# Iamdarika/Spotify_recommender

Measured on AMD Instinct MI355X. Metric: queries/sec, cosine top-100 over a 10M x 12 fp32 catalogue, higher is better.
Workload: dtype f32 (every score is the exact fp32 chain; a 12 B/row 8-bit replica only rules rows out); 1 GPU; 10000000 synthetic tracks x 12 fp32 features, top-100, 1 MI355X (BASELINE configs[2], HBM-roofline run); rows=10000000, topn=100, rows_per_gpu=10000000, lanes=2, seed=12345, generator=torch.rand(seed) uniform[0,1) on device

## Files before the change

spotify_recommender_amd/csrc/engine_single.hip.h:

```cpp
#pragma once

#include "engine_state.hip.h"

#include <type_traits>

namespace {

int flush_mstream(mi355rec* h, hipStream_t s);

bool use_half(const mi355rec* h, const uint64_t* upper_dev) {
    if (!h->d_half || upper_dev || h->replica_mode == MI355REC_REPLICA_OFF) return false;
    return h->replica_mode == MI355REC_REPLICA_ON || h->replica_mode == MI355REC_REPLICA_FP16 || h->n >= kHalfAutoMinRows;
}

bool use_q8(const mi355rec* h) { return h->d_q8 && h->replica_mode != MI355REC_REPLICA_FP16; }

int single_kind(const mi355rec* h, const uint64_t* upper_dev) {
    if (!use_half(h, upper_dev)) return kFp32;
    return use_q8(h) ? kQ8 : kFp16;
}

bool q8_exact_sample(const mi355rec* h) { return h->geom[kQ8].iters >= 3; }

constexpr int kBucketAutoMaxTopn = 128;
// ... 219 lines not shown
        L.epoch = next_epoch(h);
        if (enqueue_f32_seed(h, qptr, query12, exclude_global, topn, h->d_half_seed, h->d_lone_ctl, &h->lone_ctl_done, L.epoch, s))
            L.bound = &h->d_lone_ctl->cutoff;
        L.sample = h->d_half_seed;
    }
    const int rc = launch_scan(h, L, qptr, query12, exclude_global, topn, s);
    if (rc == MI355REC_OK && fused) *fused = L.tail.counters != nullptr;
    return rc;
}

int enqueue_merge(mi355rec* h, const uint64_t* lists, int n_lists, int list_len, int topn,
                  uint64_t* out_keys, int64_t* out_idx, float* out_score, hipStream_t s, uint32_t notify = 0) {
    const int slot = timing_begin(h, h->ev_merge, h->n_merge_pairs, h->merge_launches, s);
    hipLaunchKernelGGL(merge_kernel, dim3(1), dim3(kMergeBlock), 0, s, lists, n_lists, list_len,
                       static_cast<int64_t>(list_len), static_cast<int64_t>(0), topn, out_keys, out_idx, out_score,
                       static_cast<int64_t>(0), notify ? h->hd_done : static_cast<uint32_t*>(nullptr), notify);
    timing_end(h, h->ev_merge, h->n_merge_pairs, slot, s);
    HIP_TRY(h, hipGetLastError());
    return MI355REC_OK;
}

int check_topn(mi355rec* h, int topn, bool allow_rounds) {
    if (topn <= 0)
        return fail(h, MI355REC_ERR_INVALID_ARG, "topn must be positive, got %d", topn);
    if (!allow_rounds && topn > kMaxTopK)
        return fail(h, MI355REC_ERR_INVALID_ARG, "topn %d > %d is not supported by this call", topn, kMaxTopK);
    return MI355REC_OK;
}

bool pairs_open(const mi355rec* h);
int flush_streamed(mi355rec* h, hipStream_t s);
int enqueue_query(mi355rec* h, const float* qptr, const float* query12, int64_t exclude_global,
                  int topn_asked, uint64_t* out_keys, int64_t* out_idx, float* out_score, hipStream_t s, uint32_t notify = 0) {
    if (pairs_open(h)) {
        const int rc = flush_streamed(h, s);
        if (rc) return rc;
    }
    const int topn = static_cast<int64_t>(topn_asked) < h->n ? topn_asked : static_cast<int>(h->n);
    if (topn < topn_asked) {
        const size_t pad = static_cast<size_t>(topn_asked - topn);
        HIP_TRY(h, hipMemsetAsync(out_keys + topn, 0, pad * sizeof(uint64_t), s));
        if (out_idx) HIP_TRY(h, hipMemsetAsync(out_idx + topn, 0xff, pad * sizeof(int64_t), s));
        if (out_score) HIP_TRY(h, hipMemsetAsync(out_score + topn, 0, pad * sizeof(float), s));
    }
    for (int done = 0; done < topn; done += kMaxTopK) {
        const int k = topn - done < kMaxTopK ? topn - done : kMaxTopK;
        const uint64_t* upper = done ? out_keys + done - 1 : nullptr;
        int lists = 0;
        LoneTail lone{h->d_lone_ctr, out_keys, out_idx, out_score, h->hd_done, notify, {0u, 0u, 0u, 0u, 0u, 0u, 0u, 0u, 0u}};
        bool fused = false;
        int rc = enqueue_scan(h, qptr, query12, exclude_global, k, upper, s, &lists, (notify && h->d_lone_ctr) ? &lone : nullptr, &fused);
        if (rc) return rc;
        if (fused) {
            ++h->lone_fused;
            continue;
        }
        rc = enqueue_merge(h, h->d_block_lists, lists, k, k, out_keys + done,
                           out_idx ? out_idx + done : nullptr, out_score ? out_score + done : nullptr, s, notify);
        if (rc) return rc;
    }
    return MI355REC_OK;
}

int wait_done(mi355rec* h, uint32_t want) {
    for (uint64_t spins = 1;; ++spins) {
        if (__atomic_load_n(h->h_done, __ATOMIC_ACQUIRE) == want) return MI355REC_OK;
        __builtin_ia32_pause();
        if ((spins & 0x3ffff) == 0) {
            const hipError_t e = hipStreamQuery(h->stream);
            if (e == hipSuccess) {
                if (__atomic_load_n(h->h_done, __ATOMIC_ACQUIRE) == want) return MI355REC_OK;
                return fail(h, MI355REC_ERR_HIP, "the query's stream drained without its completion word");
            }
            if (e != hipErrorNotReady) return fail(h, MI355REC_ERR_HIP, "hipStreamQuery: %s", hipGetErrorString(e));
        }
    }
}

int ensure_streamed_alloc(mi355rec* h);
int ensure_streamed(mi355rec* h) {
    if (h->streamed_ready) return MI355REC_OK;
    const int rc = ensure_streamed_alloc(h);
    if (rc != MI355REC_OK) {
        for (int i = 0; i < 2; ++i) {
            if (h->d_stream_lists[i]) (void)hipFree(h->d_stream_lists[i]);
            h->d_stream_lists[i] = nullptr;
        }
        return rc;
    }
    h->streamed_ready = true;
    return MI355REC_OK;
}

int ensure_streamed_alloc(mi355rec* h) {
    const size_t words = static_cast<size_t>(most(h, &ScanGeom::sgrid)) * kMaxTopK;
    for (int i = 0; i < 2; ++i) HIP_TRY(h, hipMalloc(&h->d_stream_lists[i], sizeof(uint64_t) * words));
    return MI355REC_OK;
}

int merge_pending(mi355rec* h, hipStream_t s) {
    h->pending = false;
    return enqueue_merge(h, h->d_stream_lists[h->pending_buf], h->pending_lists, h->pending_topn, h->pending_topn,
                         h->pending_out, nullptr, nullptr, s);
}

int launch_stashed(mi355rec* h, hipStream_t s, bool with_next, const float* next_ptr, const float* next_q,
                   int64_t next_exclude, int next_topn, int next_buf, uint32_t next_epoch_tag);

int drain_pairs(mi355rec* h, hipStream_t s);

int flush_single_stream(mi355rec* h, hipStream_t s);
int flush_streamed(mi355rec* h, hipStream_t s) {
    const int rc = drain_pairs(h, s);
    return rc ? rc : flush_single_stream(h, s);
}

int flush_single_stream(mi355rec* h, hipStream_t s) {
    if (h->stashed.has) {
        const int rc = launch_stashed(h, s, false, nullptr, nullptr, -1, 0, 0, 0u);
        if (rc) return rc;
    }
    return h->pending ? merge_pending(h, s) : MI355REC_OK;
}

int launch_stashed(mi355rec* h, hipStream_t s, bool with_next, const float* next_ptr, const float* next_q,
                   int64_t next_exclude, int next_topn, int next_buf, uint32_t next_epoch_tag) {
    auto& st = h->stashed;
    const bool next_bucketed = with_next && use_bucket(h, st.kind, next_topn, h->geom_bucket.riders > 0);
    const ScanGeom& g = stream_geom(h, st.kind, next_bucketed);
    if (st.kind == kFp32 && h->pending && h->pending_topn > kRideTopnMax) {
        const int rc = merge_pending(h, s);
        if (rc) return rc;
    }
    ScanLaunch L;
    L.kind = st.kind;
    L.streamed = true;
    const int buf = h->pending ? 1 - h->pending_buf : 0;
    if (h->pending) L.prev = PrevMerge{h->d_stream_lists[h->pending_buf], h->pending_lists, h->pending_topn, h->pending_out};
    int scanners = g.sgrid;
    L.iters = g.siters;
    if (with_next && (g.riders > 0 || g.nbhd)) {
        scanners = g.r_scan;
        L.iters = g.r_iters;
        L.next = make_next_seed(h, st.kind, g.riders, g.nbhd, next_ptr, next_q, next_exclude, next_topn, next_epoch_tag,
                                h->d_stream_seed[next_buf], g.hoists ? h->d_stream_ctl + next_buf : nullptr, h->ctl_done[next_buf],
                                next_bucketed);
    }
    L.grid = scanners + 1 + L.next.n_wgs + L.next.nbhd;
    L.lists = h->d_stream_lists[buf];
    L.sample = h->d_stream_seed[st.seed_buf];
    L.bound = st.cutoff_ready ? &h->d_stream_ctl[st.seed_buf].cutoff : nullptr;
    L.epoch = st.epoch;
    L.bucketed = st.bucketed;
    const int rc = launch_scan(h, L, st.qptr, st.q, st.exclude, st.topn, s);
    if (rc) return rc;
    if (L.next.ctl) h->ctl_done[next_buf] += static_cast<unsigned>(L.next.n_wgs);
    h->pending = true;
    h->pending_buf = buf;
    h->pending_topn = st.topn;
    h->pending_out = st.out;
    h->pending_lists = scanners;
    st.has = false;
    return MI355REC_OK;
}

int enqueue_streamed_single(mi355rec* h, const float* qptr, const float* query12, int64_t exclude_global, int topn,
                            uint64_t* out_keys, hipStream_t s, int accepted_kind = -1) {
    int rc = MI355REC_OK;
    if (MI355REC_EXP_FLAG("MI355REC_EXP_RIDE_NOMERGE") && h->pending) {
        rc = flush_single_stream(h, s);
        if (rc) return rc;
    }
    const int kind = accepted_kind >= 0 ? accepted_kind : single_kind(h, nullptr);
    int seed_buf = 0;
    bool sampled = false, nbhd_taken = false;
    const uint32_t epoch = next_epoch(h);
    const bool bucketed = use_bucket(h, kind, topn, h->stashed.has && h->stashed.kind == kind && h->geom_bucket.riders > 0);
    const ScanGeom& ng = stream_geom(h, kind, bucketed);
    if (kind == kQ8) h->last_sample = bucketed ? MI355REC_SAMPLE_BUCKETED : MI355REC_SAMPLE_STRIDED;
    if (h->stashed.has) {
        seed_buf = 1 - h->stashed.seed_buf;
        const bool same = h->stashed.kind == kind;
        sampled = same && ng.riders > 0;
        nbhd_taken = same && ng.nbhd;
        rc = launch_stashed(h, s, same, qptr, query12, exclude_global, topn, seed_buf, epoch);
        if (rc) return rc;
    }
    bool bound_ready = sampled && ng.hoists;
    if (!sampled) {
        if (kind == kFp32) {
            if (h->n >= kF32LoneSeedMinRows)
                bound_ready = enqueue_f32_seed(h, qptr, query12, exclude_global, topn, h->d_stream_seed[seed_buf], h->d_stream_ctl + seed_buf,
                                               &h->ctl_done[seed_buf], epoch, s);
        } else if (!nbhd_taken) {
            enqueue_half_seed(h, kind, qptr, query12, exclude_global, topn, h->d_stream_seed[seed_buf], epoch, s, bucketed);
        }
        HIP_TRY(h, hipGetLastError());
    }
    auto& st = h->stashed;
    st.has = true;
    st.qptr = qptr;
    if (!qptr) std::memcpy(st.q, query12, sizeof st.q);
    st.exclude = exclude_global;
    st.topn = topn;
    st.out = out_keys;
    st.seed_buf = seed_buf;
    st.epoch = epoch;
    st.kind = kind;
    st.bucketed = bucketed;
    st.cutoff_ready = bound_ready;
    return MI355REC_OK;
}

bool pairing_on(const mi355rec* h) {
    if (h->pairing == MI355REC_PAIRING_ON || h->pairing == MI355REC_PAIRING_GROUPS) return true;
    if (h->pairing == MI355REC_PAIRING_OFF) return false;
    return h->n >= MI355REC_PAIRING_AUTO_MIN_ROWS;
}
bool groups_on(const mi355rec* h) {
    if (h->pairing == MI355REC_PAIRING_GROUPS) return true;
    return h->pairing == MI355REC_PAIRING_AUTO && h->n >= MI355REC_GROUPS_AUTO_MIN_ROWS;
}
bool pairs_open(const mi355rec* h) { return h->pairs.n_wait > 0 || h->pairs.n_form > 0 || h->pairs.n_pending > 0; }

void free_pairs(mi355rec* h) {
    auto& P = h->pairs;
    for (int i = 0; i < 8; ++i) {
        if (P.lists[i]) (void)hipFree(P.lists[i]);
        if (P.seed[i]) (void)hipFree(P.seed[i]);
        P.lists[i] = nullptr;
        P.seed[i] = nullptr;
    }
    if (P.ctl) (void)hipFree(P.ctl);
    P.ctl = nullptr;
    P.ready = false;
}

int ensure_pairs_alloc(mi355rec* h) {
    auto& P = h->pairs;
    const size_t words = static_cast<size_t>(h->geom[kQ8].grid > 0 ? h->geom[kQ8].grid : 1) * kPairMaxTopk;
    for (int i = 0; i < 8; ++i) {
        HIP_TRY(h, hipMalloc(&P.lists[i], sizeof(uint64_t) * words));
        HIP_TRY(h, hipMalloc(&P.seed[i], sizeof(unsigned long long) * kSampleSlots));
        HIP_TRY(h, hipMemset(P.seed[i], 0, sizeof(unsigned long long) * kSampleSlots));
    }
    HIP_TRY(h, hipMalloc(&P.ctl, sizeof(SeedCtl) * 8));
    HIP_TRY(h, hipMemset(P.ctl, 0, sizeof(SeedCtl) * 8));
    return MI355REC_OK;
}
int ensure_pairs(mi355rec* h) {
    if (h->pairs.ready) return MI355REC_OK;
    const int rc = ensure_pairs_alloc(h);
    if (rc != MI355REC_OK) {
        free_pairs(h);
        return rc;
    }
    for (unsigned& d : h->pairs.ctl_done) d = 0u;
    h->pairs.ready = true;
    return MI355REC_OK;
}

int merge_pair_pending(mi355rec* h, hipStream_t s) {
    auto& P = h->pairs;
    const int count = P.n_pending;
    P.n_pending = 0;
    for (int x = 0; x < count; ++x) {
        const int rc = enqueue_merge(h, P.lists[4 * P.pending_set + x], P.pending_lists, P.pending_topn, P.pending_topn, P.pending_out[x],
                                     nullptr, nullptr, s);
        if (rc) return rc;
    }
    return MI355REC_OK;
}

int launch_pairs(mi355rec* h, hipStream_t s, const mi355rec::Stashed* next, int n_next, bool next_bucketed) {
    auto& P = h->pairs;
    const int n_scan = P.n_wait;
    const int pairs = n_scan / 2;
    const int topn = P.wait[0].topn;
    if (P.n_pending) {
        bool shared = false;
        for (int x = 0; x < P.n_pending; ++x)
            for (int y = x + 1; y < P.n_pending; ++y) {
                const uint64_t* lo = P.pending_out[x] < P.pending_out[y] ? P.pending_out[x] : P.pending_out[y];
                const uint64_t* hi = P.pending_out[x] < P.pending_out[y] ? P.pending_out[y] : P.pending_out[x];
                shared = shared || hi < lo + P.pending_topn;
            }
        if (shared) {
            const int rc = merge_pair_pending(h, s);
            if (rc) return rc;
        }
    }
    const int side_queries = (pairs == 2 || P.n_pending == 4 || n_next == 4) ? 4 : 2;
    const ScanGeom& g = stream_geom(h, kQ8, n_next > 0 && next_bucketed);
    const bool riders = n_next > 0 && (g.riders > 0 || g.nbhd);
    const int extra = side_queries * (1 + (riders ? g.riders + (g.nbhd ? 1 : 0) : 0));
    const int64_t tiles = (h->n + Q8PairConfig::kTileRows - 1) / Q8PairConfig::kTileRows;
    int64_t slots = pairs == 2 ? (g.cap - extra) / 2 : g.grid - extra;
    if (slots > kRideMaxLists - 1) slots = kRideMaxLists - 1;
    if (slots > tiles) slots = tiles;
    if (pairs == 2 && slots >= 8) slots &= ~static_cast<int64_t>(7);
    if (slots < 1) slots = 1;
    const int64_t scanners = slots * pairs;
    const int iters = static_cast<int>((tiles + slots - 1) / slots);
    const int set = P.n_pending ? 1 - P.pending_set : 0;
    Q8PairSide side;
    std::memset(&side, 0, sizeof side);
    side.queries = side_queries;
    for (int x = 0; x < 4; ++x) side.prev[x] = no_prev_merge();
    for (int x = 0; x < P.n_pending; ++x)
        side.prev[x] = PrevMerge{P.lists[4 * P.pending_set + x], P.pending_lists, P.pending_topn, P.pending_out[x]};
    if (riders) {
        for (int x = 0; x < n_next; ++x)
            side.next[x] = make_next_seed(h, kQ8, g.riders, g.nbhd, next[x].qptr, next[x].q, next[x].exclude, next[x].topn, next[x].epoch,
                                          P.seed[next[x].seed_buf], g.hoists ? P.ctl + next[x].seed_buf : nullptr,
                                          P.ctl_done[next[x].seed_buf], next_bucketed);
        for (int x = n_next; x < side_queries; ++x) {
            side.next[x].n_wgs = side.next[0].n_wgs;
            side.next[x].nbhd = side.next[0].nbhd;
        }
    }
    Q8PairArgs args;
    std::memset(&args, 0, sizeof args);
    for (int x = 0; x < n_scan; ++x) {
        const mi355rec::Stashed& q = P.wait[x];
        Q8PairArg& a = args.q[x];
        a.qarg = make_query_arg(h, q.qptr, q.q);
        a.query_ptr = q.qptr;
        a.exclude_global = q.exclude;
        a.block_lists = P.lists[4 * set + x];
        a.seed_vals = P.seed[q.seed_buf];
        a.cutoff_ready = q.cutoff_ready ? &P.ctl[q.seed_buf].cutoff : nullptr;
        a.n_seed = q8_seed_count(h, q.bucketed);
        a.epoch = q.epoch;
    }
    const dim3 grid(static_cast<unsigned>(scanners + side_queries * (1 + side.next[0].n_wgs + side.next[0].nbhd)));
    LAUNCH_TIMED(h, h->ev_scan, h->n_scan_pairs, h->scan_launches, scan_q8_kernel_pair<Q8PairConfig>, grid, dim3(Q8PairConfig::kBlock), s,
                 h->d_feats, h->d_q8, h->n, iters, h->row_base, args, pairs, topn, h->d_half_rescored, side);
    HIP_TRY(h, hipGetLastError());
    h->half_scans += n_scan;
    h->q8_scans += n_scan;
    h->routes.q8 += n_scan;
    h->stream_pair_launches += pairs;
    if (pairs == 2) ++h->stream_group_launches;
    for (int x = 0; x < n_next; ++x)
        if (side.next[x].ctl) P.ctl_done[next[x].seed_buf] += static_cast<unsigned>(side.next[x].n_wgs);
    P.n_pending = n_scan;
    P.pending_set = set;
    P.pending_lists = static_cast<int>(slots);
    P.pending_topn = topn;
    for (int x = 0; x < n_scan; ++x) P.pending_out[x] = P.wait[x].out;
    P.n_wait = 0;
    return MI355REC_OK;
}

int close_forming(mi355rec* h, hipStream_t s, int count) {
    auto& P = h->pairs;
    const int topn = P.form[0].topn;
    const int set = P.n_wait ? 1 - (P.wait[0].seed_buf >> 2) : 0;
    const bool bucketed = use_bucket(h, kQ8, topn, h->geom_bucket.riders > 0);
    const ScanGeom& ng = stream_geom(h, kQ8, bucketed);
    mi355rec::Stashed nx[4];
    for (int i = 0; i < count; ++i) {
        nx[i] = P.form[i];
        nx[i].seed_buf = 4 * set + i;
        nx[i].epoch = next_epoch(h);
        nx[i].bucketed = bucketed;
    }
    h->last_sample = bucketed ? MI355REC_SAMPLE_BUCKETED : MI355REC_SAMPLE_STRIDED;
    bool sampled = false;
    if (P.n_wait) {
        sampled = ng.riders > 0;
        const int rc = launch_pairs(h, s, nx, count, bucketed);
        if (rc) return rc;
    }
    if (!sampled) {
        for (int i = 0; i < count; ++i)
            enqueue_half_seed(h, kQ8, nx[i].qptr, nx[i].q, nx[i].exclude, topn, P.seed[nx[i].seed_buf], nx[i].epoch, s, bucketed);
        HIP_TRY(h, hipGetLastError());
    }
    for (int i = 0; i < count; ++i) {
        nx[i].cutoff_ready = sampled && ng.hoists;
        P.wait[i] = nx[i];
    }
    P.n_wait = count;
    for (int i = count; i < P.n_form; ++i) P.form[i - count] = P.form[i];
    P.n_form -= count;
    return MI355REC_OK;
}

int drain_pairs(mi355rec* h, hipStream_t s) {
    auto& P = h->pairs;
    if (P.n_form >= 2) {
        const int rc = close_forming(h, s, 2);
        if (rc) return rc;
    }
    if (P.n_wait) {
        const int rc = launch_pairs(h, s, nullptr, 0, false);
        if (rc) return rc;
    }
    if (P.n_pending) {
        const int rc = merge_pair_pending(h, s);
        if (rc) return rc;
    }
    if (P.n_form) {
        const mi355rec::Stashed f = P.form[0];
        P.n_form = 0;
        return enqueue_streamed_single(h, f.qptr, f.q, f.exclude, f.topn, f.out, s, h->d_q8 ? f.kind : -1);
    }
    return MI355REC_OK;
}

int enqueue_streamed(mi355rec* h, const float* qptr, const float* query12, int64_t exclude_global, int topn,
                     uint64_t* out_keys, hipStream_t s) {
    int rc = ensure_streamed(h);
    if (rc) return rc;
    rc = flush_mstream(h, s);
    if (rc) return rc;
    auto& P = h->pairs;
    bool pair = single_kind(h, nullptr) == kQ8 && topn <= kPairMaxTopk && pairing_on(h);
    if (pair && ensure_pairs(h) != MI355REC_OK) {
        (void)hipGetLastError();
        pair = false;
    }
    if (pair && P.n_form && (P.form[0].topn != topn || P.first_replica_mode != h->replica_mode || P.first_sample_mode != h->sample_mode)) {
        rc = drain_pairs(h, s);
        if (rc) return rc;
    }
    if (!pair) {
        if (pairs_open(h)) {
            rc = drain_pairs(h, s);
            if (rc) return rc;
        }
        return enqueue_streamed_single(h, qptr, query12, exclude_global, topn, out_keys, s);
    }
    if (h->stashed.has || h->pending) {
        rc = flush_single_stream(h, s);
        if (rc) return rc;
    }
    mi355rec::Stashed x;
    x.has = true;
    x.qptr = qptr;
    if (!qptr) std::memcpy(x.q, query12, sizeof x.q);
    x.exclude = exclude_global;
    x.topn = topn;
    x.out = out_keys;
    x.kind = kQ8;
    x.by_pointer = qptr && !(qptr >= h->d_feats && qptr < h->d_feats + h->n * kDim);
    if (P.n_form >= 2 && !groups_on(h)) {
        rc = close_forming(h, s, 2);
        if (rc) return rc;
    }
    if (!P.n_form) {
        P.first_replica_mode = h->replica_mode;
        P.first_sample_mode = h->sample_mode;
    }
    P.form[P.n_form++] = x;
    if (P.n_form & 1) return MI355REC_OK;
    h->last_sample = use_bucket(h, kQ8, topn, h->geom_bucket.riders > 0) ? MI355REC_SAMPLE_BUCKETED : MI355REC_SAMPLE_STRIDED;
    bool closes = P.n_form == 4 || !groups_on(h);
    if (h->pairing == MI355REC_PAIRING_AUTO && P.n_pending == 0) closes = true;
    for (int i = 0; i < P.n_form; ++i) closes = closes || P.form[i].by_pointer;
    for (int i = 0; i < P.n_wait; ++i) closes = closes || P.wait[i].by_pointer;
    return closes ? close_forming(h, s, P.n_form) : MI355REC_OK;
}

}
```

spotify_recommender_amd/csrc/replica_q8.hip.h:

```cpp
#pragma once

#include "replica.hip.h"

#ifndef MI355_Q8_QUERY_BITS
#define MI355_Q8_QUERY_BITS 16
#endif

namespace mi355 {

constexpr int kQ8QueryBits = MI355_Q8_QUERY_BITS;
static_assert(kQ8QueryBits == 16 || kQ8QueryBits == 8, "the query is one or two int8 digits per component");
constexpr float kQ8Step = 1.0f / 254.0f;
constexpr float kQ8QueryScale = kQ8QueryBits == 16 ? 32000.0f : 127.0f;
constexpr float kQ8DotScale = 127.0f * kQ8QueryScale;
constexpr float kQ8QueryResidual = 3.4642f * 0.5f / kQ8QueryScale;
constexpr float kQ8Slack = 3e-5f;
constexpr uint32_t kQ8Special = 0x80u;


__device__ __forceinline__ void q8_pack_row(const float4& a, const float4& b, const float4& c, float tot, uint32_t& d0, uint32_t& d1,
                                            uint32_t& d2) {
    const bool valid = tot >= kBqMinNorm2 && tot <= kBqMaxNorm2;
    if (valid || tot == 0.0f) {
        const float inv = valid ? __builtin_amdgcn_rsqf(tot) * 127.0f : 0.0f;
// ... 466 lines not shown
}

template <int kBlock>
__device__ __forceinline__ void q8_ride_sample(const float* __restrict__ feats, const uint4* __restrict__ q8, int64_t n, int64_t row_base,
                                               const NextSeed& next, int rider, int* s_scratch, int* s_flag, int* s_seeds,
                                               SelectSmem& s_sel) {
    const bool bucketed = next.bucket.rows != nullptr;
    const Q8Query nq = bucketed ? q8_bucket_sample(feats, next.bucket, n, row_base, next.query_ptr, next.q, next.exclude_global,
                                                   static_cast<unsigned long long*>(next.out), next.epoch, rider, next.n_wgs,
                                                   next.debug_skip > 0, s_scratch, s_sel)
                                : q8_seed_rider(feats, q8, n, row_base, next, rider);
    const int n_vals = bucketed ? kBucketPicks * kBucketGroups : next.regions * kHalfSeedWaves;
    if (next.ctl) {
        float v;
        if (sample_arrive_and_select<kBlock>(next.ctl, next.done_base, static_cast<unsigned>(next.n_wgs),
                                             static_cast<const unsigned long long*>(next.out), n_vals, next.topk, next.epoch, s_flag,
                                             s_seeds, s_sel, s_scratch, v)) {
            const float c = !nq.ok ? -__builtin_inff() : (next.exact != 0 ? v - nq.margin : v - 2.0f * nq.margin);
            if (threadIdx.x == 0) next.ctl->cutoff = tag_value(next.epoch, __float_as_uint(c));
        }
    }
}

template <int kBlockT, int kMinWavesT, int kDepthT>
struct Q8Cfg {
    static constexpr int kBlock = kBlockT;
    static constexpr int kMinWaves = kMinWavesT;
    static constexpr int kDepth = kDepthT;
    static constexpr int kTileRows = 4 * kBlockT;
    static constexpr int kCandCap = kCandLimit + kTileRows;
    static constexpr int kCandPerThread = (kCandCap + kBlockT - 1) / kBlockT;
};
using DefaultQ8Cfg = Q8Cfg<512, 4, 2>;

template <typename Cfg, bool kQueryFromRow, bool kWithMerge, bool kLoneTail = false>
__global__ __launch_bounds__(Cfg::kBlock, Cfg::kMinWaves) void scan_q8_kernel(
    const float* __restrict__ feats, const uint4* __restrict__ q8, int64_t n, int iters, int64_t row_base,
    QueryArg qarg, const float* __restrict__ query_ptr, int64_t exclude_global, int topk, uint64_t* __restrict__ block_lists,
    const unsigned long long* __restrict__ seed_vals , int n_seed ,
    unsigned long long* __restrict__ rescored ,
    PrevMerge prev, NextSeed next, const unsigned long long* __restrict__ cutoff_ready ,
    LoneTail lone, uint32_t epoch ) {
    constexpr int kBlock = Cfg::kBlock;
    static_assert(!(kWithMerge && kLoneTail), "a streamed query's merge rides in the next launch");
    __shared__ typename std::conditional<kWithMerge || kLoneTail, HalfScanOrMergeSmem<Cfg>, HalfScanSmemT<Cfg>>::type s_mem;
    __shared__ int s_lone_flag;
    HalfScanSmemT<Cfg>* sm;
    unsigned nblocks = gridDim.x;
    unsigned vb = blockIdx.x;
    MI355REC_PHASE(0);
    if constexpr (kWithMerge) {
        const unsigned extra = 1u + static_cast<unsigned>(next.n_wgs) + static_cast<unsigned>(next.nbhd);
        nblocks = gridDim.x - extra;
        vb = blockIdx.x >= extra ? blockIdx.x - extra : nblocks + blockIdx.x;
        if (vb >= nblocks) {
            if (vb == nblocks) {
                q8_ride_merge(s_mem.merge, prev);
            } else if (next.nbhd && vb == gridDim.x - 1u) {
                q8_ride_nbhd<kBlock>(feats, n, row_base, next, reinterpret_cast<int*>(s_mem.scan.cand));
            } else {
                static_assert(kBlock == kHalfSeedBlock && sizeof(s_mem.scan.cand) >= sizeof(int) * kBucketScratch, "the riders' geometry");
                q8_ride_sample<kBlock>(feats, q8, n, row_base, next, static_cast<int>(vb - nblocks - 1u), reinterpret_cast<int*>(s_mem.scan.cand),
                                       &s_mem.scan.count, &s_mem.scan.seeds, s_mem.scan.sel);
            }
            __syncthreads();
            MI355REC_PHASE(5);
            return;
        }
        sm = &s_mem.scan;
    } else if constexpr (kLoneTail) {
        (void)next;
        sm = &s_mem.scan;
    } else {
        (void)next;
        (void)lone;
        (void)s_lone_flag;
        sm = &s_mem;
    }
    uint64_t* const s_cand = sm->cand;
    SelectSmem& s_sel = sm->sel;
    int& s_count = sm->count;

    const unsigned bid = vb;
    const int tid = threadIdx.x;
    const int lane = tid & 63;

    const int64_t n_quads = (n + 3) >> 2;
    const int64_t last_quad = n_quads - 1;
    const int64_t quad_begin = static_cast<int64_t>(bid) * kBlock + tid;
    const int64_t quad_stride = static_cast<int64_t>(nblocks) * kBlock;

    auto load_tile = [&](HalfTile& dst, int it) {
        int64_t quad = quad_begin + static_cast<int64_t>(it) * quad_stride;
        quad = quad < n_quads ? quad : last_quad;
        const uint4* p = q8 + quad * 3;
        dst.t0 = p[0];
        dst.t1 = p[1];
        dst.t2 = p[2];
    };

    constexpr int kDepth = Cfg::kDepth;
    float cutoff_left = 0.0f;
    const unsigned long long nbhd_raw = seed_vals[kNbhdSlot];
    SampleRaw sample_raw;
#pragma unroll
    for (int r = 0; r < kHalfSeedPerThread; ++r) sample_raw.t[r] = 0ull;
    const int n_sample = n_seed < 0 ? -n_seed : n_seed;
    if (cutoff_ready) {
        cutoff_left = untag_cutoff(*cutoff_ready, epoch);
    } else {
        sample_raw = sample_request<kBlock>(seed_vals, n_sample);
    }
    HalfTile ring[kDepth];
#pragma unroll
    for (int d = 0; d < kDepth - 1; ++d) load_tile(ring[d], d);
    float q[kDim];
    q8_load_query((kQueryFromRow || kWithMerge) ? query_ptr : nullptr, qarg.q, q);
    const float qn = query_norm(q);
    const Q8Query hq = q8_query(q, qn);
    const Sample sample = sample_finish(sample_raw, epoch);
    if (hq.hi[0] != 0 || n >= 0) MI355REC_PHASE(1);
    if (sample.v[0] != 0x12345u || n >= 0) MI355REC_PHASE(6);

    if (tid == 0) {
        s_count = 0;
        sm->seeds = 0;
        sm->rescored = 0;
    }
    int n_rescored = 0;
    __syncthreads();
    float cutoff;
    if (cutoff_ready) {
        cutoff = cutoff_left;
    } else {
        cutoff = q8_cutoff_from_sample<kBlock>(sample, n_sample, topk, n_seed < 0, hq, &sm->seeds, s_sel, reinterpret_cast<int*>(s_cand));
    }
    uint64_t thr = 0;
    if (const uint32_t nbv = untag_value(nbhd_raw, epoch)) {
        thr = (static_cast<uint64_t>(nbv) << 32) - 1ull;
        if (hq.ok) {
            const float nb_cut = ordered_to_score(nbv) - hq.margin;
            cutoff = nb_cut > cutoff ? nb_cut : cutoff;
        }
    }
    int cut_d = q8_threshold(cutoff);
    MI355REC_PHASE(2);
    int compact_at = 2 * topk > 256 ? 2 * topk : 256;
    if (compact_at > kCandLimit) compact_at = kCandLimit;

    Row pend;
    pend.a = pend.b = pend.c = make_float4(0.0f, 0.0f, 0.0f, 0.0f);
    int64_t pend_r = 0;
    bool pend_on = false;

    auto append = [&](bool have, const Row& row, int64_t r) {
        const float s = cosine_score(q, qn, row);
        const int64_t g = row_base + r;
        uint64_t key = pack_key(s, static_cast<uint32_t>(g));
        if (g == exclude_global) key = 0;
        const bool pass = have && key > thr;
        const uint64_t ballot = __ballot(pass);
        if (ballot) {
            int base = 0;
            if (lane == 0) base = atomicAdd(&s_count, __popcll(ballot));
            base = __builtin_amdgcn_readfirstlane(base);
            const int pos = base + lanes_below(ballot);
            if (pass) s_cand[pos] = key;
        }
    };
    auto consume = [&]() {
        if (__ballot(pend_on)) append(pend_on, pend, pend_r);
        pend_on = false;
    };

    auto process_tile = [&](const HalfTile& t, int it) {
        const int64_t quad = quad_begin + static_cast<int64_t>(it) * quad_stride;
        const int64_t r0 = quad * 4;
        int a[4];
        bool special[4];
        q8_dot4(hq, t, a, special);
        bool hit[4];
#pragma unroll
        for (int u = 0; u < 4; ++u) hit[u] = special[u] | (a[u] >= cut_d);
        const uint64_t maybe = __ballot(hit[0] | hit[1] | hit[2] | hit[3]);
        consume();
        uint32_t mask = 0u;
        if (maybe) {
            const int64_t left = n - r0;
            const int valid = quad < n_quads ? (left < 4 ? static_cast<int>(left) : 4) : 0;
#pragma unroll
            for (int u = 0; u < 4; ++u) mask |= (hit[u] && u < valid) ? (1u << u) : 0u;
        }
        const uint64_t any = maybe ? __ballot(mask != 0u) : 0ull;
        if (any) {
            n_rescored += __popcll(any);
            const int first = mask ? __builtin_ctz(mask) : 0;
            pend_r = r0 + first;
            pend = load_row(feats, mask ? pend_r : static_cast<int64_t>(0));
            pend_on = mask != 0u;
            uint32_t rest = mask & (mask - 1u);
            while (__ballot(rest != 0u)) {
                const int u = rest ? __builtin_ctz(rest) : 0;
                const bool have = rest != 0u;
                n_rescored += __popcll(__ballot(have));
                const Row extra = load_row(feats, have ? r0 + u : static_cast<int64_t>(0));
                append(have, extra, r0 + u);
                rest &= rest - 1u;
            }
        }
        __syncthreads();
        const int c = s_count;
        __syncthreads();
        if (c >= compact_at) {
            const uint64_t local_thr = compact_candidates<kBlock, Cfg::kCandPerThread>(s_cand, &s_count, topk, false, s_sel);
            if (local_thr > thr) {
                thr = local_thr;
                if (hq.ok) {
                    const float local_cut = ordered_to_score(static_cast<uint32_t>(thr >> 32)) - hq.margin;
                    cutoff = local_cut > cutoff ? local_cut : cutoff;
                    cut_d = q8_threshold(cutoff);
                }
            }
        }
    };

    for (int it = 0; it < iters; it += kDepth) {
#pragma unroll
        for (int sidx = 0; sidx < kDepth; ++sidx) {
            load_tile(ring[(sidx + kDepth - 1) % kDepth], it + sidx + kDepth - 1);
            if (it + sidx < iters) process_tile(ring[sidx], it + sidx);
        }
    }
    consume();

    if (lane == 0 && n_rescored) atomicAdd(&sm->rescored, n_rescored);
    __syncthreads();
    MI355REC_PHASE(3);
    if (tid == 0) rescored[bid] += static_cast<unsigned long long>(sm->rescored);
    if (s_count > kRankCountMax && s_count > topk)
        compact_candidates<kBlock, Cfg::kCandPerThread>(s_cand, &s_count, topk, false, s_sel);
    __syncthreads();
    block_rank_and_store<kBlock, kLoneTail>(s_cand, s_count, block_lists + static_cast<int64_t>(bid) * topk, topk);
    if constexpr (kLoneTail) lone_tail(s_mem.merge, &s_lone_flag, block_lists, topk, lone);
    __syncthreads();
    MI355REC_PHASE(4);
}

constexpr int kPairMaxTopk = 128;

__device__ __forceinline__ int q8_uniform(int v) { return __builtin_amdgcn_readfirstlane(v); }
__device__ __forceinline__ float q8_uniform(float v) { return __int_as_float(__builtin_amdgcn_readfirstlane(__float_as_int(v))); }
__device__ __forceinline__ uint64_t q8_uniform(uint64_t v) {
    const uint32_t lo = static_cast<uint32_t>(__builtin_amdgcn_readfirstlane(static_cast<int>(static_cast<uint32_t>(v))));
    const uint32_t hi = static_cast<uint32_t>(__builtin_amdgcn_readfirstlane(static_cast<int>(static_cast<uint32_t>(v >> 32))));
    return (static_cast<uint64_t>(hi) << 32) | lo;
}
__device__ __forceinline__ Q8Query q8_uniform(const Q8Query& q) {
    Q8Query r;
#pragma unroll
    for (int j = 0; j < 3; ++j) {
        r.hi[j] = q8_uniform(q.hi[j]);
        r.lo[j] = q8_uniform(q.lo[j]);
    }
    r.inv = q.inv;
    r.margin = q8_uniform(q.margin);
    r.ok = q8_uniform(q.ok ? 1 : 0) != 0;
    return r;
}
constexpr int kPairCandLimit = 2 * kPairMaxTopk;

__device__ __forceinline__ int q8_pair_neg_cut(int cut_d) { return -(cut_d > -(1 << 30) ? cut_d : -(1 << 30)); }
__device__ __forceinline__ int q8_pair_excess(const Q8Query& q, int neg_cut, uint32_t d0, uint32_t d1, uint32_t d2) {
    int hi = __builtin_amdgcn_sdot4(static_cast<int>(d0), q.hi[0], 0, false);
    hi = __builtin_amdgcn_sdot4(static_cast<int>(d1), q.hi[1], hi, false);
    hi = __builtin_amdgcn_sdot4(static_cast<int>(d2), q.hi[2], hi, false);
    if constexpr (kQ8QueryBits == 16) {
        int acc = static_cast<int>((static_cast<uint32_t>(hi) << 8) + static_cast<uint32_t>(neg_cut));
        acc = __builtin_amdgcn_sdot4(static_cast<int>(d0), q.lo[0], acc, false);
        acc = __builtin_amdgcn_sdot4(static_cast<int>(d1), q.lo[1], acc, false);
        acc = __builtin_amdgcn_sdot4(static_cast<int>(d2), q.lo[2], acc, false);
        return acc;
    } else {
        return hi + neg_cut;
    }
}
__device__ __forceinline__ void q8_pair_excess4(const Q8Query& q, int neg_cut, const HalfTile& t, int (&e)[4]) {
    e[0] = q8_pair_excess(q, neg_cut, t.t0.x, t.t0.y, t.t0.z);
    e[1] = q8_pair_excess(q, neg_cut, t.t0.w, t.t1.x, t.t1.y);
    e[2] = q8_pair_excess(q, neg_cut, t.t1.z, t.t1.w, t.t2.x);
    e[3] = q8_pair_excess(q, neg_cut, t.t2.y, t.t2.z, t.t2.w);
}

template <int kBlockT, int kMinWavesT, int kDepthT>
struct Q8PairCfg {
    static constexpr int kBlock = kBlockT;
    static constexpr int kMinWaves = kMinWavesT;
    static constexpr int kDepth = kDepthT;
    static constexpr int kTileRows = 4 * kBlockT;
    static constexpr int kCandCap = kPairCandLimit + kTileRows;
    static constexpr int kCandPerThread = (kCandCap + kBlockT - 1) / kBlockT;
};
using DefaultQ8PairCfg = Q8PairCfg<512, 4, 2>;

template <typename Cfg>
struct Q8PairSmemT {
    uint64_t cand[2][Cfg::kCandCap];
    SelectSmem sel;
    int count[2];
    int seeds[2];
    int rescored;
};
template <typename Cfg>
union Q8PairOrMergeSmem {
    Q8PairSmemT<Cfg> scan;
    MergeSmemT<Cfg::kBlock, kRideMaxLists, kHalfRideSurvCap> merge;
};

struct Q8PairArg {
    QueryArg qarg;
    const float* query_ptr;
    long long exclude_global;
    uint64_t* block_lists;
    const unsigned long long* seed_vals;
    const unsigned long long* cutoff_ready;
    int n_seed;
    uint32_t epoch;
};

struct Q8PairSide {
    PrevMerge prev[4];
    NextSeed next[4];
    int queries;
    int pad;
};

struct Q8PairArgs {
    Q8PairArg q[4];
};

template <typename Cfg>
__global__ __launch_bounds__(Cfg::kBlock, Cfg::kMinWaves) void scan_q8_kernel_pair(
    const float* __restrict__ feats, const uint4* __restrict__ q8, int64_t n, int iters, int64_t row_base, Q8PairArgs args,
    int pairs , int topk, unsigned long long* __restrict__ rescored , Q8PairSide side) {
    constexpr int kBlock = Cfg::kBlock;
    __shared__ Q8PairOrMergeSmem<Cfg> s_mem;
    const unsigned riders = static_cast<unsigned>(side.next[0].n_wgs), nbhds = static_cast<unsigned>(side.next[0].nbhd);
    const unsigned nq = static_cast<unsigned>(side.queries);
    const unsigned extra = nq * (1u + riders + nbhds);
    const unsigned nblocks = gridDim.x - extra;
    const unsigned vb = blockIdx.x >= extra ? blockIdx.x - extra : nblocks + blockIdx.x;
    if (vb >= nblocks) {
        static_assert(kBlock == kHalfSeedBlock && sizeof(s_mem.scan.cand) >= sizeof(int) * kBucketScratch &&
                          sizeof(s_mem.scan.cand) >= sizeof(int) * Nbhd<kBlock>::kScratch, "the riders' geometry");
        int* const s_scratch = reinterpret_cast<int*>(s_mem.scan.cand);
        const unsigned e = vb - nblocks;
        if (e < nq) {
            q8_ride_merge(s_mem.merge, side.prev[e]);
        } else if (e < nq + nq * riders) {
            const unsigned which = (e - nq) / riders;
            if (side.next[which].out)
                q8_ride_sample<kBlock>(feats, q8, n, row_base, side.next[which], static_cast<int>(e - nq - which * riders), s_scratch,
                                       &s_mem.scan.count[0], &s_mem.scan.seeds[0], s_mem.scan.sel);
        } else {
            const unsigned which = e - nq - nq * riders;
            if (side.next[which].out) q8_ride_nbhd<kBlock>(feats, n, row_base, side.next[which], s_scratch);
        }
        __syncthreads();
        return;
    }
    Q8PairSmemT<Cfg>* const sm = &s_mem.scan;
    SelectSmem& s_sel = sm->sel;

    unsigned group = 0u, bid = vb, slots = nblocks;
    if (pairs == 2) {
        slots = nblocks >> 1;
        if (slots >= 8u) {
            group = (vb >> 3) & 1u;
            bid = ((vb >> 4) << 3) | (vb & 7u);
        } else {
            group = vb >= slots ? 1u : 0u;
            bid = vb - group * slots;
        }
    }
    const Q8PairArg& arg_a = args.q[2u * group];
    const Q8PairArg& arg_b = args.q[2u * group + 1u];
    const int tid = threadIdx.x;
    const int lane = tid & 63;

    const int64_t n_quads = (n + 3) >> 2;
    const int64_t last_quad = n_quads - 1;
    const int64_t quad_begin = static_cast<int64_t>(bid) * kBlock + tid;
    const int64_t quad_stride = static_cast<int64_t>(slots) * kBlock;

    const int64_t last_at = last_quad * 3;
    const int64_t stride_at = quad_stride * 3;
    int64_t next_at = quad_begin * 3;
    auto load_tile = [&](HalfTile& dst, int ) {
        const uint4* p = q8 + (next_at < last_at ? next_at : last_at);
        next_at += stride_at;
        dst.t0 = p[0];
        dst.t1 = p[1];
        dst.t2 = p[2];
    };

    struct Mine {
        float q[kDim];
        float qn;
        Q8Query hq;
        float cutoff;
        uint64_t thr;
        int cut_d;
        int neg_cut;
        int n_rescored;
        uint64_t* s_cand;
        int* s_count;
    };
    Mine A, B;
    A.s_cand = sm->cand[0];
    B.s_cand = sm->cand[1];
    A.s_count = &sm->count[0];
    B.s_count = &sm->count[1];

    constexpr int kDepth = Cfg::kDepth;
    const unsigned long long nbhd_raw_a = arg_a.seed_vals[kNbhdSlot], nbhd_raw_b = arg_b.seed_vals[kNbhdSlot];
    float left_a = 0.0f, left_b = 0.0f;
    SampleRaw raw_a, raw_b;
#pragma unroll
    for (int r = 0; r < kHalfSeedPerThread; ++r) raw_a.t[r] = raw_b.t[r] = 0ull;
    const int n_sample_a = arg_a.n_seed < 0 ? -arg_a.n_seed : arg_a.n_seed, n_sample_b = arg_b.n_seed < 0 ? -arg_b.n_seed : arg_b.n_seed;
    if (arg_a.cutoff_ready) left_a = untag_cutoff(*arg_a.cutoff_ready, arg_a.epoch);
    else raw_a = sample_request<kBlock>(arg_a.seed_vals, n_sample_a);
    if (arg_b.cutoff_ready) left_b = untag_cutoff(*arg_b.cutoff_ready, arg_b.epoch);
    else raw_b = sample_request<kBlock>(arg_b.seed_vals, n_sample_b);
    HalfTile ring[kDepth];
#pragma unroll
    for (int d = 0; d < kDepth - 1; ++d) load_tile(ring[d], d);
    q8_load_query(arg_a.query_ptr, arg_a.qarg.q, A.q);
    q8_load_query(arg_b.query_ptr, arg_b.qarg.q, B.q);
    A.qn = q8_uniform(query_norm(A.q));
    B.qn = q8_uniform(query_norm(B.q));
    A.hq = q8_uniform(q8_query(A.q, A.qn));
    B.hq = q8_uniform(q8_query(B.q, B.qn));

    if (tid == 0) {
        sm->count[0] = sm->count[1] = 0;
        sm->seeds[0] = sm->seeds[1] = 0;
        sm->rescored = 0;
    }
    __syncthreads();
    auto start = [&](Mine& m, const Q8PairArg& arg, const SampleRaw& raw, int n_sample, float left, unsigned long long nbhd_raw, int* s_seeds) {
        if (arg.cutoff_ready) {
            m.cutoff = left;
        } else {
            const Sample sample = sample_finish(raw, arg.epoch);
            m.cutoff = q8_cutoff_from_sample<kBlock>(sample, n_sample, topk, arg.n_seed < 0, m.hq, s_seeds, s_sel, reinterpret_cast<int*>(m.s_cand));
        }
        m.thr = 0;
        if (const uint32_t nbv = untag_value(nbhd_raw, arg.epoch)) {
            m.thr = (static_cast<uint64_t>(nbv) << 32) - 1ull;
            if (m.hq.ok) {
                const float nb_cut = ordered_to_score(nbv) - m.hq.margin;
                m.cutoff = nb_cut > m.cutoff ? nb_cut : m.cutoff;
            }
        }
        m.cutoff = q8_uniform(m.cutoff);
        m.thr = q8_uniform(m.thr);
        m.cut_d = q8_uniform(q8_threshold(m.cutoff));
        m.neg_cut = q8_uniform(q8_pair_neg_cut(m.cut_d));
        m.n_rescored = 0;
    };
    start(A, arg_a, raw_a, n_sample_a, left_a, nbhd_raw_a, &sm->seeds[0]);
    __syncthreads();
    start(B, arg_b, raw_b, n_sample_b, left_b, nbhd_raw_b, &sm->seeds[1]);
    int compact_at = 2 * topk > 256 ? 2 * topk : 256;
    if (compact_at > kPairCandLimit) compact_at = kPairCandLimit;

    auto append = [&](Mine& m, int64_t exclude_global, bool have, const Row& row, int64_t r) {
        const float s = cosine_score(m.q, m.qn, row);
        const int64_t g = row_base + r;
        uint64_t key = pack_key(s, static_cast<uint32_t>(g));
        if (g == exclude_global) key = 0;
        const bool pass = have && key > m.thr;
        const uint64_t ballot = __ballot(pass);
        if (ballot) {
            int base = 0;
            if (lane == 0) base = atomicAdd(m.s_count, __popcll(ballot));
            base = __builtin_amdgcn_readfirstlane(base);
            const int pos = base + lanes_below(ballot);
            if (pass) m.s_cand[pos] = key;
        }
    };
    Row pend;
    pend.a = pend.b = pend.c = make_float4(0.0f, 0.0f, 0.0f, 0.0f);
    int64_t pend_r = 0;
    uint32_t pend_for = 0u;
    auto score_row = [&](uint32_t who, const Row& row, int64_t r) {
        if (__ballot((who & 1u) != 0u)) append(A, arg_a.exclude_global, (who & 1u) != 0u, row, r);
        if (__ballot((who & 2u) != 0u)) append(B, arg_b.exclude_global, (who & 2u) != 0u, row, r);
    };
    auto consume = [&]() {
        if (__ballot(pend_for != 0u)) score_row(pend_for, pend, pend_r);
        pend_for = 0u;
    };
    auto fetch = [&](uint32_t mask_a, uint32_t mask_b, int64_t r0) {
        const uint32_t both = mask_a | mask_b;
        if (!__ballot(both != 0u)) return;
        auto whose = [&](int u) { return ((mask_a >> u) & 1u) | (((mask_b >> u) & 1u) << 1); };
        auto count = [&](uint32_t who) {
            A.n_rescored += __popcll(__ballot((who & 1u) != 0u));
            B.n_rescored += __popcll(__ballot((who & 2u) != 0u));
        };
        const int first = both ? __builtin_ctz(both) : 0;
        pend_r = r0 + first;
        pend = load_row(feats, both ? pend_r : static_cast<int64_t>(0));
        pend_for = both ? whose(first) : 0u;
        count(pend_for);
        uint32_t rest = both & (both - 1u);
        while (__ballot(rest != 0u)) {
            const int u = rest ? __builtin_ctz(rest) : 0;
            const uint32_t who = rest ? whose(u) : 0u;
            count(who);
            const Row extra = load_row(feats, rest ? r0 + u : static_cast<int64_t>(0));
            score_row(who, extra, r0 + u);
            rest &= rest - 1u;
        }
    };
    auto tighten = [&](Mine& m) {
        const uint64_t local_thr = compact_candidates<kBlock, Cfg::kCandPerThread>(m.s_cand, m.s_count, topk, false, s_sel);
        if (local_thr > m.thr) {
            m.thr = q8_uniform(local_thr);
            if (m.hq.ok) {
                const float local_cut = ordered_to_score(static_cast<uint32_t>(m.thr >> 32)) - m.hq.margin;
                m.cutoff = q8_uniform(local_cut > m.cutoff ? local_cut : m.cutoff);
                m.cut_d = q8_uniform(q8_threshold(m.cutoff));
                m.neg_cut = q8_uniform(q8_pair_neg_cut(m.cut_d));
            }
        }
    };

    auto process_tile = [&](const HalfTile& t, int it) {
        const int64_t quad = quad_begin + static_cast<int64_t>(it) * quad_stride;
        const int64_t r0 = quad * 4;
        int ea[4], eb[4];
        q8_pair_excess4(A.hq, A.neg_cut, t, ea);
        q8_pair_excess4(B.hq, B.neg_cut, t, eb);
        const bool special[4] = {(t.t0.x & 0xffu) == kQ8Special, (t.t0.w & 0xffu) == kQ8Special, (t.t1.z & 0xffu) == kQ8Special,
                                 (t.t2.y & 0xffu) == kQ8Special};
        int top = ea[0] > eb[0] ? ea[0] : eb[0];
#pragma unroll
        for (int u = 1; u < 4; ++u) {
            top = ea[u] > top ? ea[u] : top;
            top = eb[u] > top ? eb[u] : top;
        }
        const uint64_t maybe = __ballot(top >= 0 || special[0] || special[1] || special[2] || special[3]);
        consume();
        if (maybe) {
            uint32_t hit_a = 0u, hit_b = 0u;
#pragma unroll
            for (int u = 0; u < 4; ++u) {
                hit_a |= (special[u] | (ea[u] >= 0)) ? (1u << u) : 0u;
                hit_b |= (special[u] | (eb[u] >= 0)) ? (1u << u) : 0u;
            }
            const int64_t left = n - r0;
            const int valid = quad < n_quads ? (left < 4 ? static_cast<int>(left) : 4) : 0;
            const uint32_t inside = (1u << valid) - 1u;
            fetch(hit_a & inside, hit_b & inside, r0);
        }
        __syncthreads();
        const int ca = *A.s_count, cb = *B.s_count;
        __syncthreads();
        if (ca >= compact_at) tighten(A);
        if (cb >= compact_at) tighten(B);
    };

    for (int it = 0; it < iters; it += kDepth) {
#pragma unroll
        for (int sidx = 0; sidx < kDepth; ++sidx) {
            load_tile(ring[(sidx + kDepth - 1) % kDepth], it + sidx + kDepth - 1);
            __builtin_amdgcn_sched_barrier(0);
            if (it + sidx < iters) process_tile(ring[sidx], it + sidx);
        }
    }
    consume();

    if (lane == 0 && A.n_rescored + B.n_rescored) atomicAdd(&sm->rescored, A.n_rescored + B.n_rescored);
    __syncthreads();
    if (tid == 0) rescored[vb] += static_cast<unsigned long long>(sm->rescored);
    auto finish = [&](Mine& m, uint64_t* block_lists) {
        if (*m.s_count > kRankCountMax && *m.s_count > topk)
            compact_candidates<kBlock, Cfg::kCandPerThread>(m.s_cand, m.s_count, topk, false, s_sel);
        __syncthreads();
        block_rank_and_store<kBlock>(m.s_cand, *m.s_count, block_lists + static_cast<int64_t>(bid) * topk, topk);
        __syncthreads();
    };
    finish(A, arg_a.block_lists);
    finish(B, arg_b.block_lists);
}

}
```

Before: 128,400 queries/s.

## Queue q8 pair-scan survivors in an LDS ring and rescore them densely

The per-thread fetch loop, which reloaded and rescored surviving rows lane by lane with divergent ballots, is replaced. Survivors for both queries are now pushed into a shared-memory ring, and the whole workgroup drains it in dense chunks: each thread loads one queued row and scores it for whichever queries flagged it. Query vectors move from registers to LDS, and the candidate lists are carved out of the existing candidate buffer. This is meant to cut wave divergence and idle lanes during fp32 rescoring. In exchange it adds atomics, extra barriers, a cap on iterations per workgroup, and an inline-asm register clobber.

New measurement: 138,100 queries/s (median of 6 runs). 1.08x the previous value.

```diff
diff --git a/spotify_recommender_amd/csrc/engine_single.hip.h b/spotify_recommender_amd/csrc/engine_single.hip.h
--- a/spotify_recommender_amd/csrc/engine_single.hip.h
+++ b/spotify_recommender_amd/csrc/engine_single.hip.h
@@ -545,6 +545,8 @@
     if (slots < 1) slots = 1;
     const int64_t scanners = slots * pairs;
     const int iters = static_cast<int>((tiles + slots - 1) / slots);
+    if (iters > kPairQueueMaxIters)
+        return fail(h, MI355REC_ERR_INVALID_ARG, "%d tiles per scanning workgroup exceed the pair scan's %d", iters, kPairQueueMaxIters);
     const int set = P.n_pending ? 1 - P.pending_set : 0;
     Q8PairSide side;
     std::memset(&side, 0, sizeof side);
diff --git a/spotify_recommender_amd/csrc/replica_q8.hip.h b/spotify_recommender_amd/csrc/replica_q8.hip.h
--- a/spotify_recommender_amd/csrc/replica_q8.hip.h
+++ b/spotify_recommender_amd/csrc/replica_q8.hip.h
@@ -792,6 +792,11 @@
 };
 using DefaultQ8PairCfg = Q8PairCfg<512, 4, 2>;
 
+constexpr int kPairRing = 4096;
+constexpr int kPairDrainAt = 64;
+constexpr int kPairQueueMaxIters = 1 << 19;
+constexpr int kPairListCap = kPairCandLimit + 2 * 512;
+
 template <typename Cfg>
 struct Q8PairSmemT {
     uint64_t cand[2][Cfg::kCandCap];
@@ -799,7 +804,10 @@
     int count[2];
     int seeds[2];
     int rescored;
+    unsigned q_tail;
+    float q[2][kDim];
 };
+static_assert((kPairRing & (kPairRing - 1)) == 0, "the ring is indexed by a mask");
 template <typename Cfg>
 union Q8PairOrMergeSmem {
     Q8PairSmemT<Cfg> scan;
@@ -860,6 +868,7 @@
     }
     Q8PairSmemT<Cfg>* const sm = &s_mem.scan;
     SelectSmem& s_sel = sm->sel;
+    asm volatile("" ::: "v118");
 
     unsigned group = 0u, bid = vb, slots = nblocks;
     if (pairs == 2) {
@@ -894,20 +903,22 @@
     };
 
     struct Mine {
-        float q[kDim];
         float qn;
         Q8Query hq;
         float cutoff;
         uint64_t thr;
         int cut_d;
         int neg_cut;
-        int n_rescored;
         uint64_t* s_cand;
         int* s_count;
     };
     Mine A, B;
-    A.s_cand = sm->cand[0];
-    B.s_cand = sm->cand[1];
+    static_assert(sizeof(sm->cand) >= 2 * kPairListCap * sizeof(uint64_t) + kPairRing * sizeof(uint32_t), "two lists and the ring");
+    static_assert(kPairListCap * sizeof(uint64_t) >= kSelScratch * sizeof(int), "a list's storage is its query's selection scratch");
+    constexpr int kListPerThread = (kPairListCap + kBlock - 1) / kBlock;
+    A.s_cand = &sm->cand[0][0];
+    B.s_cand = A.s_cand + kPairListCap;
+    uint32_t* const s_ring = reinterpret_cast<uint32_t*>(B.s_cand + kPairListCap);
     A.s_count = &sm->count[0];
     B.s_count = &sm->count[1];
 
@@ -925,17 +936,28 @@
     HalfTile ring[kDepth];
 #pragma unroll
     for (int d = 0; d < kDepth - 1; ++d) load_tile(ring[d], d);
-    q8_load_query(arg_a.query_ptr, arg_a.qarg.q, A.q);
-    q8_load_query(arg_b.query_ptr, arg_b.qarg.q, B.q);
-    A.qn = q8_uniform(query_norm(A.q));
-    B.qn = q8_uniform(query_norm(B.q));
-    A.hq = q8_uniform(q8_query(A.q, A.qn));
-    B.hq = q8_uniform(q8_query(B.q, B.qn));
+    {
+        float qa[kDim], qb[kDim];
+        q8_load_query(arg_a.query_ptr, arg_a.qarg.q, qa);
+        q8_load_query(arg_b.query_ptr, arg_b.qarg.q, qb);
+        A.qn = q8_uniform(query_norm(qa));
+        B.qn = q8_uniform(query_norm(qb));
+        A.hq = q8_uniform(q8_query(qa, A.qn));
+        B.hq = q8_uniform(q8_query(qb, B.qn));
+        if (tid == 0) {
+#pragma unroll
+            for (int j = 0; j < kDim; ++j) {
+                sm->q[0][j] = qa[j];
+                sm->q[1][j] = qb[j];
+            }
+        }
+    }
 
     if (tid == 0) {
         sm->count[0] = sm->count[1] = 0;
         sm->seeds[0] = sm->seeds[1] = 0;
         sm->rescored = 0;
+        sm->q_tail = 0u;
     }
     __syncthreads();
     auto start = [&](Mine& m, const Q8PairArg& arg, const SampleRaw& raw, int n_sample, float left, unsigned long long nbhd_raw, int* s_seeds) {
@@ -957,7 +979,6 @@
         m.thr = q8_uniform(m.thr);
         m.cut_d = q8_uniform(q8_threshold(m.cutoff));
         m.neg_cut = q8_uniform(q8_pair_neg_cut(m.cut_d));
-        m.n_rescored = 0;
     };
     start(A, arg_a, raw_a, n_sample_a, left_a, nbhd_raw_a, &sm->seeds[0]);
     __syncthreads();
@@ -965,11 +986,14 @@
     int compact_at = 2 * topk > 256 ? 2 * topk : 256;
     if (compact_at > kPairCandLimit) compact_at = kPairCandLimit;
 
-    auto append = [&](Mine& m, int64_t exclude_global, bool have, const Row& row, int64_t r) {
-        const float s = cosine_score(m.q, m.qn, row);
+    auto append = [&](Mine& m, const Q8PairArg& arg, const float* s_q, bool have, const Row& row, int64_t r) {
+        float q[kDim];
+#pragma unroll
+        for (int j = 0; j < kDim; ++j) q[j] = s_q[j];
+        const float s = cosine_score(q, m.qn, row);
         const int64_t g = row_base + r;
         uint64_t key = pack_key(s, static_cast<uint32_t>(g));
-        if (g == exclude_global) key = 0;
+        if (g == arg.exclude_global) key = 0;
         const bool pass = have && key > m.thr;
         const uint64_t ballot = __ballot(pass);
         if (ballot) {
@@ -980,43 +1004,8 @@
             if (pass) m.s_cand[pos] = key;
         }
     };
-    Row pend;
-    pend.a = pend.b = pend.c = make_float4(0.0f, 0.0f, 0.0f, 0.0f);
-    int64_t pend_r = 0;
-    uint32_t pend_for = 0u;
-    auto score_row = [&](uint32_t who, const Row& row, int64_t r) {
-        if (__ballot((who & 1u) != 0u)) append(A, arg_a.exclude_global, (who & 1u) != 0u, row, r);
-        if (__ballot((who & 2u) != 0u)) append(B, arg_b.exclude_global, (who & 2u) != 0u, row, r);
-    };
-    auto consume = [&]() {
-        if (__ballot(pend_for != 0u)) score_row(pend_for, pend, pend_r);
-        pend_for = 0u;
-    };
-    auto fetch = [&](uint32_t mask_a, uint32_t mask_b, int64_t r0) {
-        const uint32_t both = mask_a | mask_b;
-        if (!__ballot(both != 0u)) return;
-        auto whose = [&](int u) { return ((mask_a >> u) & 1u) | (((mask_b >> u) & 1u) << 1); };
-        auto count = [&](uint32_t who) {
-            A.n_rescored += __popcll(__ballot((who & 1u) != 0u));
-            B.n_rescored += __popcll(__ballot((who & 2u) != 0u));
-        };
-        const int first = both ? __builtin_ctz(both) : 0;
-        pend_r = r0 + first;
-        pend = load_row(feats, both ? pend_r : static_cast<int64_t>(0));
-        pend_for = both ? whose(first) : 0u;
-        count(pend_for);
-        uint32_t rest = both & (both - 1u);
-        while (__ballot(rest != 0u)) {
-            const int u = rest ? __builtin_ctz(rest) : 0;
-            const uint32_t who = rest ? whose(u) : 0u;
-            count(who);
-            const Row extra = load_row(feats, rest ? r0 + u : static_cast<int64_t>(0));
-            score_row(who, extra, r0 + u);
-            rest &= rest - 1u;
-        }
-    };
     auto tighten = [&](Mine& m) {
-        const uint64_t local_thr = compact_candidates<kBlock, Cfg::kCandPerThread>(m.s_cand, m.s_count, topk, false, s_sel);
+        const uint64_t local_thr = compact_candidates<kBlock, kListPerThread>(m.s_cand, m.s_count, topk, false, s_sel);
         if (local_thr > m.thr) {
             m.thr = q8_uniform(local_thr);
             if (m.hq.ok) {
@@ -1028,9 +1017,80 @@
         }
     };
 
+    static_assert(kPairDrainAt - 1 + Cfg::kTileRows <= kPairRing && kPairDrainAt <= kBlock, "what a tile can add fits the ring");
+    static_assert(kPairListCap >= kPairCandLimit + 2 * kBlock, "two chunks' keys fit a list between two looks at its count");
+    static_assert(Cfg::kTileRows == 2048, "an entry keeps the row's place in its tile in 11 bits");
+    const int wave_first = q8_uniform(tid & ~63);
+    const int64_t tile_stride = quad_stride * 4;
+    const int64_t wg_first = static_cast<int64_t>(bid) * Cfg::kTileRows;
+    uint32_t head = 0u;
+    uint32_t tail_seen = 0u;
+    int n_rescored = 0;
+    Row pend;
+    pend.a = pend.b = pend.c = make_float4(0.0f, 0.0f, 0.0f, 0.0f);
+    uint32_t pend_e = 0u;
+    uint32_t pend_n = 0u;
+
+    auto push = [&](uint32_t hit_a, uint32_t hit_b, int it) {
+        const uint32_t both = hit_a | hit_b;
+        uint64_t at[4];
+        int total = 0;
+#pragma unroll
+        for (int u = 0; u < 4; ++u) {
+            at[u] = __ballot(((both >> u) & 1u) != 0u);
+            total += __popcll(at[u]);
+        }
+        if (!total) return;
+        n_rescored += __popc(hit_a) + __popc(hit_b);
+        unsigned base = 0u;
+        if (lane == 0) base = atomicAdd(&sm->q_tail, static_cast<unsigned>(total));
+        base = static_cast<unsigned>(__builtin_amdgcn_readfirstlane(static_cast<int>(base)));
+        const uint32_t l0 = static_cast<uint32_t>(it) * Cfg::kTileRows + 4u * static_cast<uint32_t>(tid);
+#pragma unroll
+        for (int u = 0; u < 4; ++u) {
+            if (at[u]) {
+                if ((both >> u) & 1u)
+                    s_ring[(base + static_cast<unsigned>(lanes_below(at[u]))) & (kPairRing - 1)] =
+                        ((l0 + u) << 2) | ((hit_a >> u) & 1u) | (((hit_b >> u) & 1u) << 1);
+                base += static_cast<unsigned>(__popcll(at[u]));
+            }
+        }
+    };
+    auto deal = [&](uint32_t cnt) {
+        pend_n = cnt;
+        if (static_cast<uint32_t>(wave_first) < cnt) {
+            const bool have = static_cast<uint32_t>(tid) < cnt;
+            const uint32_t e = s_ring[(head + static_cast<uint32_t>(tid)) & (kPairRing - 1)];
+            pend_e = have ? e : 0u;
+            const uint32_t l = pend_e >> 2;
+            pend = load_row(feats, static_cast<int64_t>(l >> 11) * tile_stride + wg_first + static_cast<int64_t>(l & 2047u));
+        }
+        head += cnt;
+    };
+    auto consume = [&]() {
+        if (static_cast<uint32_t>(wave_first) < pend_n) {
+            const uint32_t l = pend_e >> 2;
+            const int64_t r = static_cast<int64_t>(l >> 11) * tile_stride + wg_first + static_cast<int64_t>(l & 2047u);
+            if (__ballot((pend_e & 1u) != 0u)) append(A, arg_a, sm->q[0], (pend_e & 1u) != 0u, pend, r);
+            if (__ballot((pend_e & 2u) != 0u)) append(B, arg_b, sm->q[1], (pend_e & 2u) != 0u, pend, r);
+        }
+        pend_n = 0u;
+    };
+    auto drain = [&](uint32_t tail) {
+        while (tail - head > static_cast<uint32_t>(kBlock)) {
+            deal(static_cast<uint32_t>(kBlock));
+            consume();
+            __syncthreads();
+            const int ca = *A.s_count, cb = *B.s_count;
+            __syncthreads();
+            if (ca >= compact_at) tighten(A);
+            if (cb >= compact_at) tighten(B);
+        }
+        deal(tail - head);
+        __syncthreads();
+    };
+
     auto process_tile = [&](const HalfTile& t, int it) {
-        const int64_t quad = quad_begin + static_cast<int64_t>(it) * quad_stride;
-        const int64_t r0 = quad * 4;
         int ea[4], eb[4];
         q8_pair_excess4(A.hq, A.neg_cut, t, ea);
         q8_pair_excess4(B.hq, B.neg_cut, t, eb);
@@ -1043,7 +1103,6 @@
             top = eb[u] > top ? eb[u] : top;
         }
         const uint64_t maybe = __ballot(top >= 0 || special[0] || special[1] || special[2] || special[3]);
-        consume();
         if (maybe) {
             uint32_t hit_a = 0u, hit_b = 0u;
 #pragma unroll
@@ -1051,16 +1110,20 @@
                 hit_a |= (special[u] | (ea[u] >= 0)) ? (1u << u) : 0u;
                 hit_b |= (special[u] | (eb[u] >= 0)) ? (1u << u) : 0u;
             }
-            const int64_t left = n - r0;
+            const int64_t quad = quad_begin + static_cast<int64_t>(it) * quad_stride;
+            const int64_t left = n - quad * 4;
             const int valid = quad < n_quads ? (left < 4 ? static_cast<int>(left) : 4) : 0;
             const uint32_t inside = (1u << valid) - 1u;
-            fetch(hit_a & inside, hit_b & inside, r0);
-        }
+            push(hit_a & inside, hit_b & inside, it);
+        }
+        consume();
         __syncthreads();
         const int ca = *A.s_count, cb = *B.s_count;
+        tail_seen = static_cast<uint32_t>(q8_uniform(static_cast<int>(sm->q_tail)));
         __syncthreads();
         if (ca >= compact_at) tighten(A);
         if (cb >= compact_at) tighten(B);
+        if (tail_seen - head >= static_cast<uint32_t>(kPairDrainAt)) drain(tail_seen);
     };
 
     for (int it = 0; it < iters; it += kDepth) {
@@ -1072,13 +1135,16 @@
         }
     }
     consume();
-
-    if (lane == 0 && A.n_rescored + B.n_rescored) atomicAdd(&sm->rescored, A.n_rescored + B.n_rescored);
+    drain(tail_seen);
+    consume();
+
+    n_rescored = wave_inclusive_scan(n_rescored);
+    if (lane == 63 && n_rescored) atomicAdd(&sm->rescored, n_rescored);
     __syncthreads();
     if (tid == 0) rescored[vb] += static_cast<unsigned long long>(sm->rescored);
     auto finish = [&](Mine& m, uint64_t* block_lists) {
         if (*m.s_count > kRankCountMax && *m.s_count > topk)
-            compact_candidates<kBlock, Cfg::kCandPerThread>(m.s_cand, m.s_count, topk, false, s_sel);
+            compact_candidates<kBlock, kListPerThread>(m.s_cand, m.s_count, topk, false, s_sel);
         __syncthreads();
         block_rank_and_store<kBlock>(m.s_cand, *m.s_count, block_lists + static_cast<int64_t>(bid) * topk, topk);
         __syncthreads();
```
